# irap-omp/deconv3d

Hardware: AMD Instinct MI355X
Metric: spaxel-updates/sec (MH-Gibbs) (higher is better)
Workload: dtype f64; 1 GPU; c3_300x300x128; fsf=moffat 11x11, lsf_taps=17, spaxels=90000, lsf=analytic MUSE stand-in (mpdaf absent), parallelism=1 chain, variance=per-voxel cube (heteroscedastic)

## Files before the change

__graft_entry__.py:

```python
import os
import subprocess
import sys

ROOT = os.path.dirname(os.path.abspath(__file__))
if ROOT not in sys.path:
    sys.path.insert(0, ROOT)
CSRC = os.path.join(ROOT, "deconv3d_amd", "csrc")


SOURCES = ["d3d_api.hip", "d3d_spatial.hip", "d3d_mh.hip", "d3d_sweep.hip", "d3d_post.hip", "d3d_region.hip", "d3d_search.hip", "d3d_prep.hip", "d3d_temper.hip", "d3d_robust.hip", "d3d_pred.hip", "d3d_noise.hip", "d3d_ctx.h", "d3d_kernels.h", "d3d_conv.h",
           "d3d_mh_small.h", "d3d_rng.h", "../../include/deconv3d_hip.h"]


def tree_source_hash():
    import hashlib
    h = hashlib.sha256()
    for name in SOURCES:
        with open(os.path.join(CSRC, name), "rb") as f:
            h.update(f.read())
    return h.hexdigest()[:16]


def _binary_hash(lib):
    code = ("import ctypes,sys; l=ctypes.CDLL(sys.argv[1]); "
            "l.d3d_source_hash.restype=ctypes.c_char_p; print(l.d3d_source_hash().decode())")
    try:
        return subprocess.check_output([sys.executable, "-c", code, lib],
                                       stderr=subprocess.DEVNULL).decode().strip()
    except (subprocess.CalledProcessError, OSError):
        return None


def build():
    env = dict(os.environ)
# ... 60 lines not shown
```

deconv3d_amd/csrc/d3d_api.hip:

```cpp
#include "d3d_ctx.h"

#include <dlfcn.h>

#define D3D_VERSION 300
#ifndef D3D_SOURCE_HASH
#define D3D_SOURCE_HASH "unknown"
#endif

namespace {
thread_local std::string g_err;
}

namespace d3dh {
int fail(int code, const char *fmt, ...) {
    char buf[512];
    va_list ap;
    va_start(ap, fmt);
    vsnprintf(buf, sizeof buf, fmt, ap);
    va_end(ap);
    g_err = buf;
    return code;
}
}

// ... 160 lines not shown
                    for (int x = xs; x - fhw < pt.dx1; x += c->fw) {
                        const bool is_real = y >= pt.y0 && y < pt.y1 && x >= pt.x0 && x < pt.x1 &&
                                             c->h_mask[(size_t)y * c->W + x];
                        if (!is_real) list.push_back(make_int4(y, x, 0, 0));
                    }
                if (pt.real[col] > 0) {
                    const long n_all_col =
                        ((long)list.size() - pt.off[col]) * (c->mh_zb ? (c->Dp + 255) / 256 : 1);
                    if (c->mh_zigzag && (ord & 1) && n_all_col > c->flow_grid) {
                        std::reverse(list.begin() + pt.off[col], list.begin() + pt.off[col] + pt.real[col]);
                        std::reverse(list.begin() + pt.off[col] + pt.real[col], list.end());
                    }
                    ++ord;
                }
                most = std::max(most, (int)list.size() - pt.off[col]);
            }
        pt.off[ncol] = (int)list.size();
        const long most_wgs = (long)most * (c->mh_zb ? (c->Dp + 255) / 256 : 1);
        pt.layers = (!c->mh_layers_forced && most_wgs < c->flow_grid / 2) ? 1 : c->mh_layers_cfg;
        const bool partitioned = c->tiled || !c->part_rects.empty();
        pt.wide = pt.layers == 1 && c->mh_wide && partitioned && c->Dp == 128 && most > 0 &&
                  most <= c->flow_grid / 4 && c->mh_defer == 1;
        pt.small = pt.layers == 1 && most_wgs < c->flow_grid / 2;
        pt.chain = false;
        pt.K = 0;
        pt.last_col = -1;
        for (int col = 0; col < ncol; ++col)
            if (pt.real[col] > 0) {
                ++pt.K;
                pt.last_col = col;
            }
#ifdef D3D_EXPERIMENTS
        if (!empty && pt.K > 0) {
            const int cus = c->flow_grid / 4;
            const int fhh_ = (c->fh - 1) / 2, fhw_ = (c->fw - 1) / 2;
            const int lx0 = ((0 - c->gx0) % c->fw + c->fw) % c->fw;
            pt.chain_sx0 = (pt.dx0 - fhw_) - ((((pt.dx0 - fhw_) - lx0) % c->fw + c->fw) % c->fw);
            pt.n_sy = (pt.dy1 - pt.dy0 + 2 * c->fh - 2) / c->fh;
            pt.n_sx = (pt.dx1 + fhw_ - 1 - pt.chain_sx0) / c->fw + 1;
            (void)fhh_;
            pt.chain_ns = c->fw * c->HL;
            const int nt = (pt.chain_ns + 63) / 64 * 64 + 64;
            const bool fh_ok = c->fh == 3 || c->fh == 5 || c->fh == 7 || c->fh == 9 || c->fh == 11;
            const double g_bytes = 4.0 * pt.K * pt.n_sy * pt.n_sx * c->Dp * 8.0;
            const size_t lds = d3d::mh_chain_lds_doubles(c->fw, c->Dp, c->N, ncol, pt.K, nt / 64 - 1) * 8;
            pt.chain = c->mh_chain_opt == 1 && c->mh_defer == 1 && c->Dp <= 256 && pt.layers == 1 &&
// ... 119 lines not shown
}

int d3dh::download_device_cube(d3d_ctx *c, const double *src, double *host) { return download_cube(c, src, host); }

namespace {

enum OptKind { OPT_LAUNCH = 0, OPT_MH = 1, OPT_TAPS = 2 };
struct OptDesc {
    const char *key, *env;
    int d3d_ctx::*field;
    OptKind kind;
    int lo, hi;
};
const OptDesc g_opts[] = {
    {"mh_defer", "D3D_MH_DEFER", &d3d_ctx::mh_defer_opt, OPT_MH, 0, 2},
    {"mh_zblocks", "D3D_MH_ZBLOCKS", &d3d_ctx::mh_zblocks, OPT_MH, 0, 1},
    {"mh_layers", "D3D_MH_LAYERS", &d3d_ctx::mh_layers_opt, OPT_MH, 0, d3d::MH_LAYERS},
    {"mh_wide", "D3D_MH_WIDE", &d3d_ctx::mh_wide, OPT_MH, 0, 1},
    {"mh_props", "D3D_MH_PROPS", &d3d_ctx::mh_props, OPT_LAUNCH, 0, 1},
    {"mh_small", "D3D_MH_SMALL", &d3d_ctx::mh_small, OPT_MH, 0, 2},
    {"halo_timing", "D3D_HALO_TIMING", &d3d_ctx::halo_timing, OPT_LAUNCH, 0, 1},
    {"mh_zigzag", "D3D_MH_ZIGZAG", &d3d_ctx::mh_zigzag, OPT_MH, 0, 1},
    {"mh_nt_ivar", "D3D_MH_NT_IVAR", &d3d_ctx::mh_nt_ivar_opt, OPT_MH, -1, 1},
    {"mh_nt", "D3D_MH_NT", &d3d_ctx::mh_nt_opt, OPT_MH, 0, 1024},
    {"uniform_ivar", "D3D_UNIFORM_IVAR", &d3d_ctx::uniform_fast_path, OPT_MH, 0, 1},
    {"conv_rows", "D3D_CONV_ROWS", &d3d_ctx::conv_rows, OPT_LAUNCH, 0, 1},
    {"conv_zb", "D3D_CONV_ZB", &d3d_ctx::conv_zb, OPT_LAUNCH, 0, 1},
    {"conv_hy", "D3D_CONV_HY", &d3d_ctx::conv_hy_opt, OPT_LAUNCH, 0, 1 << 20},
    {"spatial_sep", "D3D_SPATIAL_SEP", &d3d_ctx::spatial_sep, OPT_TAPS, 0, 1},
    {"sep_fuse", "D3D_SEP_FUSE", &d3d_ctx::sep_fuse, OPT_LAUNCH, 0, 1},
    {"spatial_mode", "D3D_SPATIAL_MODE", &d3d_ctx::march_mode, OPT_LAUNCH, 0, 3},
    {"march_hy", "D3D_MARCH_HY", &d3d_ctx::march_hy_opt, OPT_TAPS, 0, 1 << 20},
    {"zmajor", "D3D_ZMAJOR", &d3d_ctx::zmajor, OPT_LAUNCH, 0, 1},
    {"zmajor_hy", "D3D_ZMAJOR_HY", &d3d_ctx::zmajor_hy, OPT_LAUNCH, 0, 1 << 20},
    {"spectral_dense", "D3D_SPECTRAL_DENSE", &d3d_ctx::spectral_dense, OPT_LAUNCH, 0, 1},
    {"spectral_blocks", "D3D_SPECTRAL_BLOCKS", &d3d_ctx::spectral_blocks, OPT_LAUNCH, 0, 1},
    {"lines_dense", "D3D_LINES_DENSE", &d3d_ctx::lines_dense, OPT_LAUNCH, 0, 3},
    {"lines_rounds", "D3D_LINES_ROUNDS", &d3d_ctx::lines_rounds, OPT_LAUNCH, 0, 64},
    {"spatial_nt", "D3D_SPATIAL_NT", &d3d_ctx::sp_nt_opt, OPT_LAUNCH, 0, 1024},
    {"xcd_remap", "D3D_XCD_REMAP", &d3d_ctx::xcd_remap, OPT_LAUNCH, 0, 1},
    {"alt_dir", "D3D_ALT_DIR", &d3d_ctx::alt_dir, OPT_LAUNCH, 0, 1},
    {"stagger", "D3D_STAGGER", &d3d_ctx::stagger, OPT_LAUNCH, 0, 1 << 20},
    {"post_nt", "D3D_POST_NT", &d3d_ctx::post_nt, OPT_LAUNCH, 0, 1},
    {"noise_timing", "D3D_NOISE_TIMING", &d3d_ctx::noise_timing, OPT_LAUNCH, 0, 1},
#ifdef D3D_EXPERIMENTS
    {"mh_chain", "D3D_MH_CHAIN", &d3d_ctx::mh_chain_opt, OPT_MH, 0, 1},
// ... 166 lines not shown
    CTX_TRY(hipMemsetAsync(c->accepted, 0, sizeof(unsigned long long), c->stream));
    CTX_TRY(hipMemsetAsync(c->acc_map, 0, (size_t)c->HW * sizeof(unsigned), c->stream));
    CTX_TRY(hipMemsetAsync(c->mask, 1, (size_t)c->HW, c->stream));
    CTX_TRY(hipStreamSynchronize(c->stream));
#undef CTX_TRY
    c->h_mask.assign((size_t)c->HW, 1);
    c->h_user_mask.assign((size_t)c->HW, 1);
    *out = c;
    return D3D_OK;
}

int d3d_ctx_destroy(d3d_ctx *c) {
    if (!c) return D3D_OK;
    (void)hipSetDevice(c->device);
    if (c->stream) (void)hipStreamSynchronize(c->stream);
    if (c->comm && g_rccl.CommDestroy) (void)g_rccl.CommDestroy(c->comm);
    c->comm = nullptr;
    for (int b = 0; b < d3d_ctx::STREAM_NB; ++b) {
        if (c->snap_host[b]) (void)hipHostFree(c->snap_host[b]);
        if (c->snap_ready[b]) (void)hipEventDestroy(c->snap_ready[b]);
        if (c->snap_done[b]) (void)hipEventDestroy(c->snap_done[b]);
    }
    if (c->copy_stream) (void)hipStreamDestroy(c->copy_stream);
    for (hipEvent_t e : c->halo_ev) (void)hipEventDestroy(e);
    if (c->ev0) (void)hipEventDestroy(c->ev0);
    if (c->ev1) (void)hipEventDestroy(c->ev1);
    if (c->own_stream) (void)hipStreamDestroy(c->own_stream);
    delete c;
    return D3D_OK;
}

int d3d_ctx_set_stream(d3d_ctx *c, void *hip_stream) {
    NEED(c, D3D_ERR_INVALID, "ctx is NULL");
    HIP_TRY(hipStreamSynchronize(c->stream));
    c->stream = hip_stream ? (hipStream_t)hip_stream : c->own_stream;
    return D3D_OK;
}

int d3d_sync(d3d_ctx *c) {
    NEED(c, D3D_ERR_INVALID, "ctx is NULL");
    HIP_TRY(hipStreamSynchronize(c->stream));
    return D3D_OK;
}

int d3d_timer_start(d3d_ctx *c) {
    NEED(c, D3D_ERR_INVALID, "ctx is NULL");
// ... 58 lines not shown
        long n = 0;
        for (const d3d_ctx::Part &pt : c->parts) n += pt.chain ? 1 : 0;
        *value = c->have_data ? n : 0;
        return D3D_OK;
    }
    if (!strcmp(key, "search_bank_ns") || !strcmp(key, "search_kernel_ns")) {
        *value = key[7] == 'b' ? c->search_bank_ns : c->search_kernel_ns;
        return D3D_OK;
    }
    if (!strcmp(key, "prep_median_ns") || !strcmp(key, "prep_stats_ns")) {
        *value = key[5] == 'm' ? c->prep_median_ns : c->prep_stats_ns;
        return D3D_OK;
    }
    if (!strcmp(key, "noise_sums_ns") || !strcmp(key, "noise_draw_ns") || !strcmp(key, "noise_apply_ns")) {
        *value = c->noise_ns[key[6] == 's' ? 0 : key[6] == 'd' ? 1 : 2];
        return D3D_OK;
    }
    if (!strcmp(key, "device_bytes")) {
        *value = (long)d3dh::dev_bytes.load();
        return D3D_OK;
    }
    if (!strcmp(key, "mh_nt_ivar_on")) {
        *value = c->mh_nt_ivar ? 1 : 0;
        return D3D_OK;
    }
    if (!strcmp(key, "batch_layers")) {
        *value = c->batch_layers;
        return D3D_OK;
    }
    if (!strcmp(key, "lsf_fits")) {
        *value = (c->have_taps && (c->ntaps == 0 || c->lsf_dense_any)) ? 1 : 0;
        return D3D_OK;
    }
    if (!strcmp(key, "lsf_taps")) {
        *value = c->ntaps;
        return D3D_OK;
    }
    if (!strcmp(key, "spatial_path") || !strcmp(key, "spectral_path") || !strcmp(key, "stage_path")) {
        *value = key[2] == 'a' ? (key[3] == 't' ? c->spatial_path : c->stage_path) : c->spectral_path;
        return D3D_OK;
    }
    if (!strcmp(key, "small_parts")) {
        long n = 0;
        for (const d3d_ctx::Part &pt : c->parts) n += d3dh::mh_part_uses_tables(c, pt) ? 1 : 0;
        *value = c->have_data ? n : 0;
        return D3D_OK;
// ... 1308 lines not shown
```

deconv3d_amd/csrc/d3d_ctx.h:

```cpp
#pragma once
#include <hip/hip_runtime.h>
#include <rccl/rccl.h>

#include <algorithm>
#include <atomic>
#include <cmath>
#include <cstdarg>
#include <cstdio>
#include <cstdlib>
#include <cstring>
#include <mutex>
#include <new>
#include <string>
#include <utility>
#include <vector>

#include "../../include/deconv3d_hip.h"
#include "d3d_kernels.h"

#ifndef D3D_WIDE_NS
#define D3D_WIDE_NS 704
#endif
constexpr int MH_WIDE_NS = D3D_WIDE_NS;
constexpr int MH_CHAIN_NT = 768;

namespace d3dh {
int fail(int code, const char *fmt, ...);
}

#define HIP_TRY(expr)                                                                   \
    do {                                                                                \
        hipError_t e_ = (expr);                                                         \
        if (e_ != hipSuccess)                                                           \
            return d3dh::fail(D3D_ERR_HIP, "%s failed: %s (%s:%d)", #expr, hipGetErrorString(e_), \
                              __FILE__, __LINE__);                                      \
    } while (0)

#define NEED(cond, code, ...) \
    do {                      \
        if (!(cond)) return d3dh::fail(code, __VA_ARGS__); \
    } while (0)

namespace d3dh {
inline std::atomic<size_t> dev_bytes{0};
}

template <typename T>
// ... 53 lines not shown
    DevBuf<double> fsf;
    DevBuf<int> lsf_shift;
    DevBuf<double> lsf_weight;
    int ntaps = 0;
    DevBuf<double> dlog;
    DevBuf<double> hwbuf;
    DevBuf<double> scal;
    DevBuf<unsigned long long> accepted;
    DevBuf<unsigned> acc_map;
    DevBuf<int4> spx;
    std::vector<int> colour_real;
    struct Part {
        int y0 = 0, y1 = 0, x0 = 0, x1 = 0;
        int dy0 = 0, dy1 = 0, dx0 = 0, dx1 = 0;
        int phase = 0;
        int layers = 1;
        bool wide = false;
        bool small = false;
        bool chain = false;
        int chain_ns = 0, chain_sx0 = 0, n_sy = 0, n_sx = 0, K = 0;
        int last_col = -1;
        std::vector<int> off;
        std::vector<int> real;
    };
    std::vector<Part> parts;
    std::vector<int4> part_rects;
    std::vector<int> part_phase;
    int n_phases = 1;
    int pend_part = -1;
    struct HaloEntry {
        int peer = 0, what = 0;
        int sy0 = 0, sy1 = 0, sx0 = 0, sx1 = 0;
        int ry0 = 0, ry1 = 0, rx0 = 0, rx1 = 0;
        size_t send_off = 0, send_n = 0, recv_off = 0, recv_n = 0;
    };
    std::vector<std::vector<HaloEntry>> plans;
    DevBuf<double> halo_send, halo_recv;
    static constexpr int STREAM_NB = 4;
    hipStream_t copy_stream = nullptr;
    DevBuf<double> snap_dev[STREAM_NB];
    double *snap_host[STREAM_NB] = {};
    hipEvent_t snap_ready[STREAM_NB] = {}, snap_done[STREAM_NB] = {};
    ncclComm_t comm = nullptr;
    int comm_rank = -1, comm_size = 0;
    int halo_timing = 0;
    static constexpr size_t HALO_RING = 64;
    std::vector<hipEvent_t> halo_ev;
    size_t halo_ev_used = 0, halo_ev_head = 0;
    double halo_ms = 0.0;
    long halo_count = 0;
    std::vector<uint8_t> h_mask;
    std::vector<uint8_t> h_user_mask;

    d3d::LineShape line = {1, {0.0, 0.0, 0.0, 0.0}, {1.0, 0.0, 0.0, 0.0}, nullptr, 0, 0.0, 0.0};
    DevBuf<double> line_tab;
    std::vector<double> h_line_tab;
    double line_tab_flux = 0.0;
    bool have_taps = false, have_data = false, have_params = false, have_cfg = false;
    bool err_valid = false;
    double min_b[3] = {}, max_b[3] = {}, amp[3] = {};
    double ra = 0;
    uint64_t seed = 0;
    int refresh_every = 1000;
    uint32_t sweep_origin = 0;

    int mh_nt = 0, mh_maxit = 0;
    int mh_nt_opt = 0, mh_maxit_opt = -1;
    int mh_defer = 1;
    int mh_defer_opt = 1;
    int mh_zblocks = 1;
    bool mh_zb = false;
    DevBuf<double> z_part;
    DevBuf<double> z_E;
#ifdef D3D_EXPERIMENTS
    DevBuf<unsigned long long> stampbuf;
    size_t stamp_launches = 0, stamp_next = 0, stamp_stride = 0;
#endif
    bool ivar_is_uniform = false;
    double ivar_uniform = 0.0;
    int uniform_fast_path = 1;
    DevBuf<double> gbuf[4];
    int lay_n = 0, lay_cy[3] = {-1, -1, -1}, lay_cx[3] = {-1, -1, -1}, lay_g[3] = {0, 0, 0};
    int mh_layers = 2;
    int batch_layers = 0;
    bool mh_nt_ivar = false;
    int mh_nt_ivar_opt = -1;
    int mh_zigzag = 1;
    int mh_layers_opt = 0;
    int mh_layers_cfg = 2;
    bool mh_layers_forced = false;
    int mh_flow = 0;
    int flow_K = 0, flow_LY = 0, flow_LX = 0, flow_items = 0, flow_grid = 0;
    int flow_last_cy = -1, flow_last_cx = -1;
    int mh_chain_opt = 0;
    DevBuf<int2> chain_cols;
    DevBuf<unsigned> chain_flags;
    DevBuf<double> chain_G;
    unsigned chain_base = 0;
    bool chain_used = false;
    int mh_props = 1;
    DevBuf<d3d::MHProposal> props;
    long props_sweep = -1;
    int mh_prio = 0;
    int mh_small = 1;
// ... 182 lines not shown
bool post_due(const d3d_ctx *c, int s);
int post_reset(d3d_ctx *c);
int region_members(d3d_ctx *c);
bool plan_has_entries(const d3d_ctx *c, int plan);
int halo_exchange(d3d_ctx *c, int plan);
int download_device_cube(d3d_ctx *c, const double *src, double *host);

bool robust_due(const d3d_ctx *c, int s);
int robust_after_sweep(d3d_ctx *c, int s);

constexpr int NOISE_STREAMS = 1024;
bool noise_due(const d3d_ctx *c, int s);
int noise_after_sweep(d3d_ctx *c, int s);

int pred_sample(d3d_ctx *c);

void colour_residue(const d3d_ctx *c, int col, int *cy, int *cx);

void pend_clear(d3d_ctx *c);
int pend_free_buf(const d3d_ctx *c);
void pend_push(d3d_ctx *c, int cy, int cx, int g);
void fill_mh_args(d3d_ctx *c, d3d::MHArgs &P);
int launch_mh(d3d_ctx *c, const d3d::MHArgs &P, unsigned grid, uint32_t sweep);
int launch_mh_zb(d3d_ctx *c, d3d::MHArgs &P, unsigned n_items, uint32_t sweep, int layers);
int launch_mh_batch(d3d_ctx *c, const d3d::MHArgs &P, unsigned grid, uint32_t sweep, int layers);
void fill_chain_args(const d3d_ctx *c, d3d::MHChainArgs &B, bool tables);
int launch_mh_defer(d3d_ctx *c, const d3d::MHArgs &P, unsigned grid, uint32_t sweep, int layers,
                    bool wide);
int flush_pending(d3d_ctx *c);
int ensure_proposals(d3d_ctx *c, uint32_t sweep);
int ensure_tables(d3d_ctx *c, bool lines);
int ensure_ptab(d3d_ctx *c);
int launch_line_table(d3d_ctx *c, const d3d::MHArgs &P, uint32_t sweep, const d3d::MHChainArgs *chains, int R);
bool mh_small_usable(const d3d_ctx *c);
int mh_ptab_row(const d3d_ctx *c, int ly, int lx, int layer = 0);
bool mh_part_uses_tables(const d3d_ctx *c, const d3d_ctx::Part &pt);
#ifdef D3D_EXPERIMENTS
int launch_mh_chain(d3d_ctx *c, int pi, uint32_t sweep0, int n_sweeps);
#endif
int launch_apply_updates(d3d_ctx *c, const d3d::MHArgs &P, const double *rec, int n);
int launch_rtnorm(d3d_ctx *c, long n, double lo, double hi, double mu, double sigma, uint64_t seed,
                  int wave_mode, double *buf);
int launch_philox(d3d_ctx *c, long n, const uint32_t *counters, const uint32_t *keys, uint32_t *words,
                  double *pairs);
#ifdef D3D_EXPERIMENTS
int launch_mh_flow(d3d_ctx *c, uint32_t sweep);
int launch_mh_pair(d3d_ctx *c, int ka, uint32_t sweep);
#endif

int temper_round(d3d_temper *t, int64_t round);
bool ctx_is_tempered(const d3d_ctx *c);
// ... 3 lines not shown
```

deconv3d_amd/csrc/d3d_mh.hip:

```cpp
#include "d3d_ctx.h"
#include "d3d_mh_small.h"

namespace d3dh {

using namespace d3d;

void pend_clear(d3d_ctx *c) {
    c->lay_n = 0;
    c->pend_part = -1;
}

int pend_free_buf(const d3d_ctx *c) {
    for (int b = 0; b < 4; ++b) {
        bool used = false;
        for (int j = 0; j < c->lay_n; ++j) used = used || c->lay_g[j] == b;
        if (!used) return b;
    }
    return 0;
}

void pend_push(d3d_ctx *c, int cy, int cx, int g) {
    c->lay_cy[c->lay_n] = cy;
    c->lay_cx[c->lay_n] = cx;
    c->lay_g[c->lay_n] = g;
// ... 353 lines not shown
    return launch_mh_small_t<UV, 256, 2, K, 1, true, false>(c, P, grid, sweep);
}
#endif

template <bool UV>
int launch_mh_small(d3d_ctx *c, const d3d::MHArgs &P, unsigned grid, uint32_t sweep, bool wide, int layers,
                    bool full) {
    NEED(P.n_lay <= layers && layers <= 2 && P.ltab && P.props, D3D_ERR_STATE,
         "internal: k_mh_small with %d pending layers of %d", P.n_lay, layers);
#ifdef D3D_EXPERIMENTS
    if (full) return launch_mh_small_full<UV, 4>(c, P, grid, sweep, layers);
#else
    (void)full;
#endif
    NEED(layers == 1, D3D_ERR_STATE, "internal: the small form keeps one pending layer");
    if (wide) return launch_mh_small_t<UV, MH_WIDE_NS, (MH_WIDE_NS > 512 ? 6 : 8), 1>(c, P, grid, sweep);
    if (c->Dp <= 64) return launch_mh_small_t<UV, 256, 8, 1>(c, P, grid, sweep);
    if (c->Dp <= 128) return launch_mh_small_t<UV, 256, 8, 2>(c, P, grid, sweep);
    return launch_mh_small_t<UV, 256, 8, 4>(c, P, grid, sweep);
}

template <bool UV>
int launch_mh_ws(d3d_ctx *c, const d3d::MHArgs &P, unsigned grid, uint32_t sweep, int layers,
                 bool wide) {
    const bool small = UV || grid < (unsigned)c->flow_grid / 2;
    if (P.ltab && layers <= 2)
        return launch_mh_small<UV>(c, P, grid, sweep, wide, layers, !(grid < (unsigned)c->flow_grid / 2));
    if (c->Dp > 256) {
        bool ntv = false;
        if constexpr (!UV) ntv = c->mh_nt_ivar && !(grid < (unsigned)c->flow_grid / 2);
        const bool few = grid < (unsigned)c->flow_grid / 2;
        if (layers >= 2) {
            if (few) return launch_mh_ws_um<UV, 4, 2, 4, false, 512>(c, P, grid, sweep);
            if constexpr (!UV)
                if (ntv) return launch_mh_ws_um<UV, 4, 2, 4, true, 512>(c, P, grid, sweep);
            return launch_mh_ws_um<UV, 4, 2, 4, false, 512>(c, P, grid, sweep);
        }
        if (few) return launch_mh_ws_um<UV, 4, 1, 4, false, 512>(c, P, grid, sweep);
        if constexpr (!UV)
            if (ntv) return launch_mh_ws_um<UV, 1, 1, 4, true, 512>(c, P, grid, sweep);
        return launch_mh_ws_um<UV, 1, 1, 4, false, 512>(c, P, grid, sweep);
    }
    if constexpr (!UV) {
        if (c->mh_nt_ivar && !small) {
            if (layers >= 3) return launch_mh_ws_um<UV, 2, 3, 2, true>(c, P, grid, sweep);
            if (layers == 2) {
                if (c->Dp > 160) return launch_mh_ws_um<UV, 2, 2, 4, true>(c, P, grid, sweep);
                return launch_mh_ws_um<UV, 2, 2, 2, true>(c, P, grid, sweep);
            }
            return launch_mh_ws_um<UV, 1, 1, 4, true>(c, P, grid, sweep);
        }
    }
    if (layers >= 3) {
        if (small) return launch_mh_ws_um<UV, 4, 3, 2>(c, P, grid, sweep);
// ... 91 lines not shown
    for (int b = 0; b < 4; ++b) {
        bool used = b == ga;
        for (int j = 0; j < c->lay_n; ++j) used = used || c->lay_g[j] == b;
        if (!used) gb = b;
    }
    F.G_a = c->gbuf[ga];
    F.G_b = c->gbuf[gb];
    c->pair_tickets += (unsigned)(F.n_a + F.n_b);
    const bool uv = c->ivar_is_uniform && c->uniform_fast_path;
    int rc;
    if (c->Dp > 160)
        rc = uv ? launch_mh_pair_t<true, 4, 4>(c, P, F, sweep) : launch_mh_pair_t<false, 2, 4>(c, P, F, sweep);
    else
        rc = uv ? launch_mh_pair_t<true, 4, 2>(c, P, F, sweep) : launch_mh_pair_t<false, 2, 2>(c, P, F, sweep);
    if (rc) return rc;
    c->lay_n = 0;
    pend_push(c, c->flow_colour[ka + 1] / c->fw, c->flow_colour[ka + 1] % c->fw, gb);
    c->pend_part = 0;
    return 0;
}
#endif

template <bool UV>
int launch_mh_zb_t(d3d_ctx *c, const d3d::MHArgs &P, unsigned n_items, uint32_t sweep, int layers) {
    constexpr int NS = 256;
    const int db = P.z_db;
    const unsigned grid = n_items * (unsigned)P.z_nb;
    const bool few = grid < (unsigned)c->flow_grid / 2;
    auto go = [&](auto kern, int M) {
        const size_t lds =
            d3d::mh_ws_lds_doubles(NS, db / 2, db, db + 2 * d3d::LSF_RL, P.npos, M) * sizeof(double);
        hipLaunchKernelGGL(kern, dim3(grid), dim3(NS + 64), lds, c->stream, P, sweep);
    };
    const bool ntv = !UV && c->mh_nt_ivar && !few;
    const int nl = P.n_lay;
    if (layers >= 2) {
        if (few) {
            if (nl == 0) go(mh_ws_kernel<NS, UV, 4, 2, 4, 0, false, true>(d3d::line_multi(P.line), false), 2);
            else if (nl == 1) go(mh_ws_kernel<NS, UV, 4, 2, 4, 1, false, true>(d3d::line_multi(P.line), false), 2);
            else go(mh_ws_kernel<NS, UV, 4, 2, 4, 2, false, true>(d3d::line_multi(P.line), false), 2);
        } else if (ntv) {
            if constexpr (!UV) {
                if (nl == 0) go(mh_ws_kernel<NS, UV, 2, 2, 4, 0, true, true>(d3d::line_multi(P.line), false), 2);
                else if (nl == 1) go(mh_ws_kernel<NS, UV, 2, 2, 4, 1, true, true>(d3d::line_multi(P.line), false), 2);
                else go(mh_ws_kernel<NS, UV, 2, 2, 4, 2, true, true>(d3d::line_multi(P.line), false), 2);
            }
        } else {
            if (nl == 0) go(mh_ws_kernel<NS, UV, 2, 2, 4, 0, false, true>(d3d::line_multi(P.line), false), 2);
            else if (nl == 1) go(mh_ws_kernel<NS, UV, 2, 2, 4, 1, false, true>(d3d::line_multi(P.line), false), 2);
            else go(mh_ws_kernel<NS, UV, 2, 2, 4, 2, false, true>(d3d::line_multi(P.line), false), 2);
        }
    } else {
        if (nl == 0) go(mh_ws_kernel<NS, UV, 4, 1, 4, 0, false, true>(d3d::line_multi(P.line), false), 1);
        else go(mh_ws_kernel<NS, UV, 4, 1, 4, 1, false, true>(d3d::line_multi(P.line), false), 1);
    }
    HIP_TRY(hipGetLastError());
    const int nw = P.z_nb * (NS / 64);
    const size_t lds2 = ((size_t)8 * nw + 8 + 16) * sizeof(double);
    hipLaunchKernelGGL(P.prior ? &d3d::k_mh_zdecide<true> : &d3d::k_mh_zdecide<false>, dim3(n_items), dim3(256), lds2,
                       c->stream, P, sweep, NS / 64);
    HIP_TRY(hipGetLastError());
    return 0;
}

int launch_mh_zb(d3d_ctx *c, d3d::MHArgs &P, unsigned n_items, uint32_t sweep, int layers) {
    NEED(P.n_lay <= (layers >= 2 ? 2 : 1), D3D_ERR_STATE, "internal: %d pending layers for the z-blocked kernel",
         P.n_lay);
    const size_t max_items = (size_t)(c->H / c->fh + 2) * (c->W / c->fw + 2);
    NEED((size_t)n_items <= max_items, D3D_ERR_STATE, "internal: %u windows in one colour launch", n_items);
    if (!c->z_part) HIP_TRY(c->z_part.alloc(max_items * P.z_nb * 32));
    if (!c->z_E) HIP_TRY(c->z_E.alloc((size_t)2 * c->slots * c->Dp));
    P.z_part = c->z_part;
    P.z_E = c->z_E;
    if (c->ivar_is_uniform && c->uniform_fast_path) return launch_mh_zb_t<true>(c, P, n_items, sweep, layers);
    return launch_mh_zb_t<false>(c, P, n_items, sweep, layers);
}

template <bool UV>
int launch_mh_batch_t(d3d_ctx *c, const d3d::MHArgs &P, unsigned grid, uint32_t sweep, int layers) {
    constexpr int NS = 256;
    const bool few = grid < (unsigned)c->flow_grid / 2;
    if (P.ltab && layers == 1) {
        const size_t lds = d3d::mh_small_lds_doubles(NS, c->HL, c->Dp, P.npos, 1) * sizeof(double);
        auto go_small = [&](auto kern) { hipLaunchKernelGGL(kern, dim3(grid), dim3(NS), lds, c->stream, P, sweep); };
        if (P.prior) {
            if (c->Dp <= 64) go_small(d3d::k_mh_small<NS, UV, 8, 1, true, 1, false, false, true>);
            else if (c->Dp <= 128) go_small(d3d::k_mh_small<NS, UV, 8, 2, true, 1, false, false, true>);
            else go_small(d3d::k_mh_small<NS, UV, 8, 4, true, 1, false, false, true>);
        } else if (c->Dp <= 64) go_small(d3d::k_mh_small<NS, UV, 8, 1, true>);
        else if (c->Dp <= 128) go_small(d3d::k_mh_small<NS, UV, 8, 2, true>);
        else go_small(d3d::k_mh_small<NS, UV, 8, 4, true>);
        HIP_TRY(hipGetLastError());
        return 0;
    }
    auto go = [&](auto kern, int M) {
        const size_t lds = d3d::mh_ws_lds_doubles(NS, c->HL, c->Dp, c->N, P.npos, M) * sizeof(double);
        hipLaunchKernelGGL(kern, dim3(grid), dim3(NS + 64), lds, c->stream, P, sweep);
    };
// ... 2 lines not shown
        if (few) {
            if (nl == 0) go(mh_ws_kernel<NS, UV, 4, 2, 2, 0, false, false, true>(d3d::line_multi(P.line), P.prior != 0), 2);
            else if (nl == 1) go(mh_ws_kernel<NS, UV, 4, 2, 2, 1, false, false, true>(d3d::line_multi(P.line), P.prior != 0), 2);
            else go(mh_ws_kernel<NS, UV, 4, 2, 2, 2, false, false, true>(d3d::line_multi(P.line), P.prior != 0), 2);
        } else {
            if (nl == 0) go(mh_ws_kernel<NS, UV, 2, 2, 2, 0, false, false, true>(d3d::line_multi(P.line), P.prior != 0), 2);
            else if (nl == 1) go(mh_ws_kernel<NS, UV, 2, 2, 2, 1, false, false, true>(d3d::line_multi(P.line), P.prior != 0), 2);
            else go(mh_ws_kernel<NS, UV, 2, 2, 2, 2, false, false, true>(d3d::line_multi(P.line), P.prior != 0), 2);
        }
    } else {
        if (nl == 0) go(mh_ws_kernel<NS, UV, 4, 1, 4, 0, false, false, true>(d3d::line_multi(P.line), P.prior != 0), 1);
        else go(mh_ws_kernel<NS, UV, 4, 1, 4, 1, false, false, true>(d3d::line_multi(P.line), P.prior != 0), 1);
    }
    HIP_TRY(hipGetLastError());
    return 0;
}

int launch_mh_batch(d3d_ctx *c, const d3d::MHArgs &P, unsigned grid, uint32_t sweep, int layers) {
    if (c->ivar_is_uniform && c->uniform_fast_path) return launch_mh_batch_t<true>(c, P, grid, sweep, layers);
    return launch_mh_batch_t<false>(c, P, grid, sweep, layers);
}

int launch_mh_defer(d3d_ctx *c, const d3d::MHArgs &P, unsigned grid, uint32_t sweep, int layers,
                    bool wide) {
    if (c->mh_defer == 1 && c->Dp <= d3d::MH_WS_MAX_DP) {
        if (c->ivar_is_uniform && c->uniform_fast_path)
            return launch_mh_ws<true>(c, P, grid, sweep, layers, wide);
        return launch_mh_ws<false>(c, P, grid, sweep, layers, wide);
    }
    switch (c->mh_nt) {
        case 128: return launch_mh_defer_nt<128>(c, P, grid, sweep);
        case 256: return launch_mh_defer_nt<256>(c, P, grid, sweep);
        case 512: return launch_mh_defer_nt<512>(c, P, grid, sweep);
        default: return launch_mh_defer_nt<1024>(c, P, grid, sweep);
    }
}

int ensure_tables(d3d_ctx *c, bool lines) {
    if (!c->props) HIP_TRY(c->props.alloc((size_t)c->HW));
    if (lines && !c->ltab) HIP_TRY(c->ltab.alloc((size_t)c->HW * 2 * c->Dp));
    return 0;
}

int launch_line_table(d3d_ctx *c, const d3d::MHArgs &P, uint32_t sweep, const d3d::MHChainArgs *chains, int R) {
    const long n = (long)(c->oy1 - c->oy0) * (c->ox1 - c->ox0) * std::max(R, 1);
    if (n <= 0) return 0;
    const size_t lds = (size_t)4 * 2 * c->N * sizeof(double);
    hipLaunchKernelGGL(d3d::line_multi(c->line) ? &d3d::k_mh_line_table<true> : &d3d::k_mh_line_table<false>,
                       dim3((unsigned)((n + 3) / 4)), dim3(256), lds, c->stream, P, sweep, c->oy0, c->oy1,
                       c->ox0, c->ox1, c->props, c->ltab, chains, R);
    HIP_TRY(hipGetLastError());
// ... 183 lines not shown
```

deconv3d_amd/csrc/d3d_sweep.hip:

```cpp
#include "d3d_ctx.h"

using namespace d3dh;

void d3dh::colour_residue(const d3d_ctx *c, int col, int *cy, int *cx) {
    *cy = ((col / c->fw - c->gy0) % c->fh + c->fh) % c->fh;
    *cx = ((col % c->fw - c->gx0) % c->fw + c->fw) % c->fw;
}

namespace {

struct SnapQueue {
    int slot[d3d_ctx::STREAM_NB];
    int head = 0, count = 0;
};

int snap_setup(d3d_ctx *c) {
    if (c->copy_stream) return 0;
    HIP_TRY(hipStreamCreateWithFlags(&c->copy_stream, hipStreamNonBlocking));
    const size_t bytes = (size_t)c->HW * 4 * sizeof(double);
    for (int b = 0; b < d3d_ctx::STREAM_NB; ++b) {
        HIP_TRY(c->snap_dev[b].alloc((size_t)c->HW * 4));
        HIP_TRY(hipHostMalloc((void **)&c->snap_host[b], bytes, hipHostMallocDefault));
        HIP_TRY(hipEventCreateWithFlags(&c->snap_ready[b], hipEventDisableTiming));
        HIP_TRY(hipEventCreateWithFlags(&c->snap_done[b], hipEventDisableTiming));
// ... 57 lines not shown
                      d3d::MHArgs &P) {
    fill_mh_args(c, P);
    P.spx = c->spx + pt.off[col];
    P.rev = (c->mh_zigzag && (ka & 1)) ? 1 : 0;
    if (tables) P.props = c->props;
    if (tables > 1) {
        P.ltab = c->ltab;
        P.ptab = c->ptab;
        int ly, lx;
        colour_residue(c, col, &ly, &lx);
        for (int j = 0; j < 2; ++j) P.ptab_row[j] = mh_ptab_row(c, ly, lx, j);
    }
    if (layers) P.write_back = (c->lay_n >= layers) ? 1 : 0;
}

void push_colour_layer(d3d_ctx *c, int pi, int col, int g, bool wrote_back) {
    if (wrote_back) c->lay_n = 0;
    int cy, cx;
    colour_residue(c, col, &cy, &cx);
    pend_push(c, cy, cx, g);
    c->pend_part = pi;
}

struct Batch {
    d3d_ctx **cs;
    int R, layers;
    bool small;
    const d3d::MHChainArgs *dev;
};

int run_part(d3d_ctx *c, int pi, uint32_t sweep, const Batch *b = nullptr) {
    d3d_ctx::Part &pt = c->parts[pi];
    const int ncol = c->fh * c->fw;
    const int layers = b ? b->layers : pt.layers;
    d3d_ctx *const self[1] = {c};
    d3d_ctx *const *cs = b ? b->cs : self;
    const bool partitioned = c->tiled || c->parts.size() > 1;
    const bool deferred =
        c->mh_defer &&
        (!partitioned || (c->mh_defer == 1 && (c->Dp <= d3d::MH_WS_MAX_DP || c->mh_zb)));
    if (c->lay_n && (c->pend_part != pi || !deferred || c->lay_n > layers))
        if (int rc = flush_pending(c)) return rc;
#ifdef D3D_EXPERIMENTS
    if (deferred && pt.chain && !b) return launch_mh_chain(c, pi, sweep, 1);
#endif
    const bool pairs = !b && deferred && c->mh_pair && !partitioned && c->mh_defer == 1 && c->Dp <= 256 &&
                       pt.layers == 2 && c->flow_K > 1 && !c->flow_first.empty();
    const bool small = deferred && c->mh_defer == 1 && !c->mh_zb && d3dh::mh_part_uses_tables(c, pt);
    const int tables = b ? (b->small ? 2 : 0)
                         : (c->mh_props && deferred && (c->mh_zb || (pt.layers == 1 && !c->deep) || small))
                               ? (small ? 2 : 1) : 0;
    int ord = 0;
    for (int col = 0; col < ncol; ++col) {
        const int n_real = pt.real[col];
        if (n_real <= 0) continue;
        const int ka = ord++;
        if (deferred) c->pend_part = pi;
#ifdef D3D_EXPERIMENTS
        if (pairs && c->lay_n == 1 && ka + 1 < c->flow_K) {
            if (c->stampbuf) goto single;
            int rc = launch_mh_pair(c, ka, sweep);
            if (rc) return rc;
            ++col;
            while (col < ncol && pt.real[col] <= 0) ++col;
            ++ord;
            continue;
        }
    single:
#else
        (void)pairs;
#endif
        if (tables && !b)
            if (int rc = ensure_proposals(c, sweep)) return rc;
        d3d::MHArgs P;
        fill_colour_args(c, pt, col, ka, deferred ? layers : 0, tables, P);
        if (!deferred) {
            if (int rc = launch_mh(c, P, (unsigned)n_real, sweep)) return rc;
            continue;
        }
        const int n_all = pt.off[col + 1] - pt.off[col];
#ifdef D3D_EXPERIMENTS
        if (!b && c->stampbuf && c->stamp_next < c->stamp_launches && (size_t)n_all * 8 <= c->stamp_stride)
            P.stamp = c->stampbuf + (c->stamp_next++) * c->stamp_stride;
#endif
        const int g_cur = pend_free_buf(c);
        int rc;
        if (b) {
            P.batch = b->dev;
            P.b_items = n_all;
            P.b_gcur = g_cur;
            for (int j = 0; j < 3; ++j) P.b_lay_g[j] = j < c->lay_n ? c->lay_g[j] : 0;
            rc = launch_mh_batch(c, P, (unsigned)n_all * b->R, sweep, layers);
        } else {
            rc = c->mh_zb ? launch_mh_zb(c, P, (unsigned)n_all, sweep, layers)
                          : launch_mh_defer(c, P, (unsigned)n_all, sweep, layers, pt.wide);
        }
        if (rc) return rc;
        for (int r = 0; r < (b ? b->R : 1); ++r) push_colour_layer(cs[r], pi, col, g_cur, P.write_back);
    }
    return 0;
}

int run_phase(d3d_ctx *c, int phase, uint32_t sweep) {
    for (size_t pi = 0; pi < c->parts.size(); ++pi)
        if (c->parts[pi].phase == phase)
            if (int rc = run_part(c, (int)pi, sweep)) return rc;
    return 0;
}

int end_sweep(d3d_ctx *c, int s, int keep_one_in, SnapQueue &snaps, double *chain_out, double *dlog_out) {
    if (s % keep_one_in == 0 && (chain_out || dlog_out))
        if (int rc = snap_push(c, snaps, s / keep_one_in, chain_out, dlog_out)) return rc;
    if (post_due(c, s))
        if (int rc = post_sample(c)) return rc;
    if (int rc = adapt_after_sweep(c, s)) return rc;
    if (c->refresh_every > 0 && s % c->refresh_every == 0) {
        if (plan_has_entries(c, D3D_PLAN_PARAMS)) {
            NEED(c->comm, D3D_ERR_STATE, "parameter gather needs d3d_comm_init");
            if (int rc = halo_exchange(c, D3D_PLAN_PARAMS)) return rc;
        }
        if (int rc = forward_into(c, c->slot[D3D_SLOT_ERR], true)) return rc;
    }
    if (int rc = robust_after_sweep(c, s)) return rc;
    return noise_after_sweep(c, s);
}

int halo_drain_one(d3d_ctx *c) {
    const size_t at = c->halo_ev_head;
    float f = 0.f;
// ... 53 lines not shown
        if (chain_batches) {
            int last = first_sweep + n_sweeps - 1;
            for (int t = s; t <= last; ++t) {
                const bool saved = t % keep_one_in == 0 && (chain_out || dlog_out);
                const bool refresh = c->refresh_every > 0 && t % c->refresh_every == 0;
                if (saved || refresh || post_due(c, t) || robust_due(c, t) || noise_due(c, t)) {
                    last = t;
                    break;
                }
            }
            if (c->lay_n && c->pend_part != 0)
                if (int rc = flush_pending(c)) return rc;
            if (int rc = launch_mh_chain(c, 0, rs, last - s + 1)) return rc;
            s = last;
        } else if (flow) {
            c->pend_part = 0;
            int rc = launch_mh_flow(c, rs);
            if (rc) return rc;
            c->pend_part = 0;
        } else
#endif
        {
            for (int ph = 0; ph < n_phases; ++ph) {
                int rc = run_phase(c, ph, rs);
                if (rc) return rc;
                if (plan_has_entries(c, ph)) {
                    hipEvent_t ev[2] = {nullptr, nullptr};
                    if (c->halo_timing) {
                        if (c->halo_ev_used == d3d_ctx::HALO_RING)
                            if (int rc2 = halo_drain_one(c)) return rc2;
                        const size_t at = (c->halo_ev_head + c->halo_ev_used) % d3d_ctx::HALO_RING;
                        while (c->halo_ev.size() < 2 * (at + 1)) {
                            hipEvent_t e;
                            HIP_TRY(hipEventCreate(&e));
                            c->halo_ev.push_back(e);
                        }
                        ev[0] = c->halo_ev[2 * at];
                        ev[1] = c->halo_ev[2 * at + 1];
                        ++c->halo_ev_used;
                        HIP_TRY(hipEventRecord(ev[0], c->stream));
                    }
                    rc = halo_exchange(c, ph);
                    if (rc) return rc;
                    if (ev[1]) HIP_TRY(hipEventRecord(ev[1], c->stream));
                }
            }
        }
// ... 136 lines not shown
}

int d3d_mh_phase(d3d_ctx *c, int phase, int sweep) {
    NEED(c, D3D_ERR_INVALID, "ctx is NULL");
    NEED(chain_ready(c), D3D_ERR_STATE, "taps/data/parameters/mh_config not set");
    NEED(phase >= 0 && phase < D3D_PLAN_PARAMS && sweep >= 0, D3D_ERR_INVALID,
         "phase %d / sweep %d out of range", phase, sweep);
    if (int rc = begin_sweeps(c, false)) return rc;
    return run_phase(c, phase, (uint32_t)sweep + c->sweep_origin);
}

int d3d_mh_colour(d3d_ctx *c, int colour, int sweep) {
    NEED(c, D3D_ERR_INVALID, "ctx is NULL");
    NEED(chain_ready(c), D3D_ERR_STATE, "taps/data/parameters/mh_config not set");
    NEED(colour >= 0 && colour < c->fh * c->fw && sweep >= 0, D3D_ERR_INVALID,
         "colour %d / sweep %d out of range", colour, sweep);
    if (int rc = begin_sweeps(c, false)) return rc;
    if (int rc = flush_pending(c)) return rc;
    for (const d3d_ctx::Part &pt : c->parts) {
        const int n_real = pt.real[colour];
        if (n_real <= 0) continue;
        d3d::MHArgs P;
        fill_colour_args(c, pt, colour, active_ordinal(pt, colour), 0, 0, P);
        int rc = launch_mh(c, P, (unsigned)n_real, (uint32_t)sweep + c->sweep_origin);
        if (rc) return rc;
    }
    return D3D_OK;
}

}
```

Measured before the change: 18.70 million spaxel-updates/s.

## Split colour launches into row strips run concurrently on auxiliary streams

Adds a strip planner that divides lattice rows into weight-balanced horizontal strips. Within each colour row, per-strip MH kernel launches are forked onto auxiliary HIP streams with separate G buffers and joined when the colour row changes. This lets independent windows from different strips overlap, aiming at the serialized per-colour launch chain on a single stream. The cost is extra events, stream synchronisation and more launches, and correctness depends on strips not interacting within one colour row.

```diff
diff --git a/__graft_entry__.py b/__graft_entry__.py
--- a/__graft_entry__.py
+++ b/__graft_entry__.py
@@ -9,7 +9,7 @@
 
 
 SOURCES = ["d3d_api.hip", "d3d_spatial.hip", "d3d_mh.hip", "d3d_sweep.hip", "d3d_post.hip", "d3d_region.hip", "d3d_search.hip", "d3d_prep.hip", "d3d_temper.hip", "d3d_robust.hip", "d3d_pred.hip", "d3d_noise.hip", "d3d_ctx.h", "d3d_kernels.h", "d3d_conv.h",
-           "d3d_mh_small.h", "d3d_rng.h", "../../include/deconv3d_hip.h"]
+           "d3d_mh_small.h", "d3d_rng.h", "../../include/deconv3d_hip.h", "d3d_strips.h"]
 
 
 def tree_source_hash():
diff --git a/deconv3d_amd/csrc/d3d_api.hip b/deconv3d_amd/csrc/d3d_api.hip
--- a/deconv3d_amd/csrc/d3d_api.hip
+++ b/deconv3d_amd/csrc/d3d_api.hip
@@ -206,6 +206,39 @@
         pt.wide = pt.layers == 1 && c->mh_wide && partitioned && c->Dp == 128 && most > 0 &&
                   most <= c->flow_grid / 4 && c->mh_defer == 1;
         pt.small = pt.layers == 1 && most_wgs < c->flow_grid / 2;
+        pt.strips = 1;
+        pt.soff.clear();
+        pt.sreal.clear();
+        {
+            const bool uv = c->ivar_is_uniform && c->uniform_fast_path;
+            const int want = c->mh_strips_opt >= 2 ? c->mh_strips_opt
+                             : (c->mh_strips_opt == 0 && most_wgs >= c->flow_grid / 2 && !uv) ? MH_STRIPS_AUTO : 1;
+            d3d_strips::Plan plan;
+            if (want >= 2 && !empty && !partitioned && c->mh_defer == 1 && (c->Dp <= d3d::MH_WS_MAX_DP || c->mh_zb) &&
+                !d3dh::mh_part_uses_tables(c, pt) && !c->mh_chain_opt && !c->mh_flow && !c->mh_pair &&
+                d3d_strips::plan(c->H, c->fh, want, &plan)) {
+                pt.strips = plan.S;
+                pt.soff.assign((size_t)ncol * (plan.S + 1), 0);
+                pt.sreal.assign((size_t)ncol * plan.S, 0);
+                for (int col = 0; col < ncol; ++col) {
+                    const int cy = col / c->fw;
+                    auto key = [&](const int4 &e) {
+                        return 2 * d3d_strips::strip_of_row(plan, d3d_strips::lattice_row(e.x, cy, c->fh)) + (e.z ? 0 : 1);
+                    };
+                    const auto b = list.begin() + pt.off[col], e = list.begin() + pt.off[col + 1];
+                    for (auto it = b; it != e; ++it)
+                        if (key(*it) < 0) return fail(D3D_ERR_HIP, "internal: lattice row outside the strips");
+                    std::stable_sort(b, e, [&](const int4 &p, const int4 &q) { return key(p) < key(q); });
+                    int *so = &pt.soff[(size_t)col * (plan.S + 1)];
+                    for (auto it = b; it != e; ++it) {
+                        const int k = key(*it);
+                        ++so[k / 2 + 1];
+                        if (!(k & 1)) ++pt.sreal[(size_t)col * plan.S + k / 2];
+                    }
+                    for (int s = 0; s < plan.S; ++s) so[s + 1] += so[s];
+                }
+            }
+        }
         pt.chain = false;
         pt.K = 0;
         pt.last_col = -1;
@@ -371,6 +404,7 @@
     {"halo_timing", "D3D_HALO_TIMING", &d3d_ctx::halo_timing, OPT_LAUNCH, 0, 1},
     {"mh_zigzag", "D3D_MH_ZIGZAG", &d3d_ctx::mh_zigzag, OPT_MH, 0, 1},
     {"mh_nt_ivar", "D3D_MH_NT_IVAR", &d3d_ctx::mh_nt_ivar_opt, OPT_MH, -1, 1},
+    {"mh_strips", "D3D_MH_STRIPS", &d3d_ctx::mh_strips_opt, OPT_MH, 0, d3d_strips::MAX_STRIPS},
     {"mh_nt", "D3D_MH_NT", &d3d_ctx::mh_nt_opt, OPT_MH, 0, 1024},
     {"uniform_ivar", "D3D_UNIFORM_IVAR", &d3d_ctx::uniform_fast_path, OPT_MH, 0, 1},
     {"conv_rows", "D3D_CONV_ROWS", &d3d_ctx::conv_rows, OPT_LAUNCH, 0, 1},
@@ -583,6 +617,11 @@
         if (c->snap_done[b]) (void)hipEventDestroy(c->snap_done[b]);
     }
     if (c->copy_stream) (void)hipStreamDestroy(c->copy_stream);
+    for (int a = 0; a < d3d_ctx::STRIP_AUX; ++a) {
+        if (c->strip_stream[a]) (void)hipStreamDestroy(c->strip_stream[a]);
+        if (c->strip_join[a]) (void)hipEventDestroy(c->strip_join[a]);
+    }
+    if (c->strip_fork) (void)hipEventDestroy(c->strip_fork);
     for (hipEvent_t e : c->halo_ev) (void)hipEventDestroy(e);
     if (c->ev0) (void)hipEventDestroy(c->ev0);
     if (c->ev1) (void)hipEventDestroy(c->ev1);
@@ -687,6 +726,10 @@
     }
     if (!strcmp(key, "mh_nt_ivar_on")) {
         *value = c->mh_nt_ivar ? 1 : 0;
+        return D3D_OK;
+    }
+    if (!strcmp(key, "mh_strips_on")) {
+        *value = (c->have_data && c->parts.size() == 1 && c->parts[0].strips > 1) ? c->parts[0].strips : 0;
         return D3D_OK;
     }
     if (!strcmp(key, "batch_layers")) {
diff --git a/deconv3d_amd/csrc/d3d_ctx.h b/deconv3d_amd/csrc/d3d_ctx.h
--- a/deconv3d_amd/csrc/d3d_ctx.h
+++ b/deconv3d_amd/csrc/d3d_ctx.h
@@ -17,12 +17,14 @@
 
 #include "../../include/deconv3d_hip.h"
 #include "d3d_kernels.h"
+#include "d3d_strips.h"
 
 #ifndef D3D_WIDE_NS
 #define D3D_WIDE_NS 704
 #endif
 constexpr int MH_WIDE_NS = D3D_WIDE_NS;
 constexpr int MH_CHAIN_NT = 768;
+constexpr int MH_STRIPS_AUTO = 2;
 
 namespace d3dh {
 int fail(int code, const char *fmt, ...);
@@ -122,6 +124,9 @@
         int last_col = -1;
         std::vector<int> off;
         std::vector<int> real;
+        int strips = 1;
+        std::vector<int> soff;
+        std::vector<int> sreal;
     };
     std::vector<Part> parts;
     std::vector<int4> part_rects;
@@ -141,6 +146,10 @@
     DevBuf<double> snap_dev[STREAM_NB];
     double *snap_host[STREAM_NB] = {};
     hipEvent_t snap_ready[STREAM_NB] = {}, snap_done[STREAM_NB] = {};
+    static constexpr int STRIP_AUX = 3;
+    hipStream_t strip_stream[STRIP_AUX] = {};
+    hipEvent_t strip_fork = nullptr, strip_join[STRIP_AUX] = {};
+    int mh_strips_opt = 0;
     ncclComm_t comm = nullptr;
     int comm_rank = -1, comm_size = 0;
     int halo_timing = 0;
@@ -179,7 +188,8 @@
     bool ivar_is_uniform = false;
     double ivar_uniform = 0.0;
     int uniform_fast_path = 1;
-    DevBuf<double> gbuf[4];
+    static constexpr int GBUFS = 8;
+    DevBuf<double> gbuf[GBUFS];
     int lay_n = 0, lay_cy[3] = {-1, -1, -1}, lay_cx[3] = {-1, -1, -1}, lay_g[3] = {0, 0, 0};
     int mh_layers = 2;
     int batch_layers = 0;
@@ -408,11 +418,12 @@
 void pend_push(d3d_ctx *c, int cy, int cx, int g);
 void fill_mh_args(d3d_ctx *c, d3d::MHArgs &P);
 int launch_mh(d3d_ctx *c, const d3d::MHArgs &P, unsigned grid, uint32_t sweep);
-int launch_mh_zb(d3d_ctx *c, d3d::MHArgs &P, unsigned n_items, uint32_t sweep, int layers);
+int launch_mh_zb(d3d_ctx *c, d3d::MHArgs &P, unsigned n_items, uint32_t sweep, int layers, unsigned total = 0,
+                 unsigned item0 = 0);
 int launch_mh_batch(d3d_ctx *c, const d3d::MHArgs &P, unsigned grid, uint32_t sweep, int layers);
 void fill_chain_args(const d3d_ctx *c, d3d::MHChainArgs &B, bool tables);
 int launch_mh_defer(d3d_ctx *c, const d3d::MHArgs &P, unsigned grid, uint32_t sweep, int layers,
-                    bool wide);
+                    bool wide, unsigned total = 0);
 int flush_pending(d3d_ctx *c);
 int ensure_proposals(d3d_ctx *c, uint32_t sweep);
 int ensure_tables(d3d_ctx *c, bool lines);
diff --git a/deconv3d_amd/csrc/d3d_mh.hip b/deconv3d_amd/csrc/d3d_mh.hip
--- a/deconv3d_amd/csrc/d3d_mh.hip
+++ b/deconv3d_amd/csrc/d3d_mh.hip
@@ -399,14 +399,14 @@
 
 template <bool UV>
 int launch_mh_ws(d3d_ctx *c, const d3d::MHArgs &P, unsigned grid, uint32_t sweep, int layers,
-                 bool wide) {
-    const bool small = UV || grid < (unsigned)c->flow_grid / 2;
+                 bool wide, unsigned total) {
+    const bool few = total < (unsigned)c->flow_grid / 2;
+    const bool small = UV || few;
     if (P.ltab && layers <= 2)
-        return launch_mh_small<UV>(c, P, grid, sweep, wide, layers, !(grid < (unsigned)c->flow_grid / 2));
+        return launch_mh_small<UV>(c, P, grid, sweep, wide, layers, !few);
     if (c->Dp > 256) {
         bool ntv = false;
-        if constexpr (!UV) ntv = c->mh_nt_ivar && !(grid < (unsigned)c->flow_grid / 2);
-        const bool few = grid < (unsigned)c->flow_grid / 2;
+        if constexpr (!UV) ntv = c->mh_nt_ivar && !few;
         if (layers >= 2) {
             if (few) return launch_mh_ws_um<UV, 4, 2, 4, false, 512>(c, P, grid, sweep);
             if constexpr (!UV)
@@ -544,11 +544,11 @@
 #endif
 
 template <bool UV>
-int launch_mh_zb_t(d3d_ctx *c, const d3d::MHArgs &P, unsigned n_items, uint32_t sweep, int layers) {
+int launch_mh_zb_t(d3d_ctx *c, const d3d::MHArgs &P, unsigned n_items, uint32_t sweep, int layers, unsigned total) {
     constexpr int NS = 256;
     const int db = P.z_db;
     const unsigned grid = n_items * (unsigned)P.z_nb;
-    const bool few = grid < (unsigned)c->flow_grid / 2;
+    const bool few = total * (unsigned)P.z_nb < (unsigned)c->flow_grid / 2;
     auto go = [&](auto kern, int M) {
         const size_t lds =
             d3d::mh_ws_lds_doubles(NS, db / 2, db, db + 2 * d3d::LSF_RL, P.npos, M) * sizeof(double);
@@ -585,17 +585,20 @@
     return 0;
 }
 
-int launch_mh_zb(d3d_ctx *c, d3d::MHArgs &P, unsigned n_items, uint32_t sweep, int layers) {
+int launch_mh_zb(d3d_ctx *c, d3d::MHArgs &P, unsigned n_items, uint32_t sweep, int layers, unsigned total,
+                 unsigned item0) {
+    if (!total) total = n_items;
     NEED(P.n_lay <= (layers >= 2 ? 2 : 1), D3D_ERR_STATE, "internal: %d pending layers for the z-blocked kernel",
          P.n_lay);
     const size_t max_items = (size_t)(c->H / c->fh + 2) * (c->W / c->fw + 2);
-    NEED((size_t)n_items <= max_items, D3D_ERR_STATE, "internal: %u windows in one colour launch", n_items);
+    NEED((size_t)item0 + n_items <= max_items, D3D_ERR_STATE, "internal: %u windows in one colour launch",
+         item0 + n_items);
     if (!c->z_part) HIP_TRY(c->z_part.alloc(max_items * P.z_nb * 32));
     if (!c->z_E) HIP_TRY(c->z_E.alloc((size_t)2 * c->slots * c->Dp));
-    P.z_part = c->z_part;
+    P.z_part = c->z_part + (size_t)item0 * P.z_nb * 32;
     P.z_E = c->z_E;
-    if (c->ivar_is_uniform && c->uniform_fast_path) return launch_mh_zb_t<true>(c, P, n_items, sweep, layers);
-    return launch_mh_zb_t<false>(c, P, n_items, sweep, layers);
+    if (c->ivar_is_uniform && c->uniform_fast_path) return launch_mh_zb_t<true>(c, P, n_items, sweep, layers, total);
+    return launch_mh_zb_t<false>(c, P, n_items, sweep, layers, total);
 }
 
 template <bool UV>
@@ -644,11 +647,12 @@
 }
 
 int launch_mh_defer(d3d_ctx *c, const d3d::MHArgs &P, unsigned grid, uint32_t sweep, int layers,
-                    bool wide) {
+                    bool wide, unsigned total) {
+    if (!total) total = grid;
     if (c->mh_defer == 1 && c->Dp <= d3d::MH_WS_MAX_DP) {
         if (c->ivar_is_uniform && c->uniform_fast_path)
-            return launch_mh_ws<true>(c, P, grid, sweep, layers, wide);
-        return launch_mh_ws<false>(c, P, grid, sweep, layers, wide);
+            return launch_mh_ws<true>(c, P, grid, sweep, layers, wide, total);
+        return launch_mh_ws<false>(c, P, grid, sweep, layers, wide, total);
     }
     switch (c->mh_nt) {
         case 128: return launch_mh_defer_nt<128>(c, P, grid, sweep);
diff --git a/deconv3d_amd/csrc/d3d_strips.h b/deconv3d_amd/csrc/d3d_strips.h
--- /dev/null
+++ b/deconv3d_amd/csrc/d3d_strips.h
@@ -0,0 +1,64 @@
+#pragma once
+
+namespace d3d_strips {
+
+constexpr int MAX_STRIPS = 4;
+constexpr int MIN_ROWS = 2;
+constexpr int ROWS_BEGIN = -1;
+
+struct Plan {
+    int S = 0;
+    int first[MAX_STRIPS + 1] = {};
+};
+
+inline int rows_end(int H, int fh) { return (H - 1 + (fh - 1) / 2) / fh + 1; }
+
+inline int lattice_row(int y, int cy, int fh) {
+    const int d = y - cy;
+    return d >= 0 ? d / fh : -((-d + fh - 1) / fh);
+}
+
+inline long row_weight(int H, int fh, int i) {
+    const int fhh = (fh - 1) / 2;
+    long w = 0;
+    for (int cy = 0; cy < fh; ++cy) {
+        const int y = cy + fh * i;
+        const int lo = y - fhh > 0 ? y - fhh : 0, hi = y + fhh < H - 1 ? y + fhh : H - 1;
+        if (hi >= lo) w += hi - lo + 1;
+    }
+    return w;
+}
+
+inline bool plan(int H, int fh, int S, Plan *out) {
+    *out = Plan();
+    if (H < 1 || fh < 1 || S < 2 || S > MAX_STRIPS) return false;
+    const int end = rows_end(H, fh);
+    if (end - ROWS_BEGIN < MIN_ROWS * S) return false;
+    long total = 0;
+    for (int i = ROWS_BEGIN; i < end; ++i) total += row_weight(H, fh, i);
+    out->first[0] = ROWS_BEGIN;
+    long cum = 0;
+    int at = ROWS_BEGIN;
+    for (int s = 1; s < S; ++s) {
+        const int lo = out->first[s - 1] + MIN_ROWS, hi = end - MIN_ROWS * (S - s);
+        while (at < lo) cum += row_weight(H, fh, at++);
+        while (at < hi) {
+            const long w = row_weight(H, fh, at);
+            if (2 * S * (cum + w) - 2 * s * total > 2 * s * total - 2 * S * cum) break;
+            cum += w;
+            ++at;
+        }
+        out->first[s] = at;
+    }
+    out->first[S] = end;
+    out->S = S;
+    return true;
+}
+
+inline int strip_of_row(const Plan &p, int i) {
+    for (int s = 0; s < p.S; ++s)
+        if (i >= p.first[s] && i < p.first[s + 1]) return s;
+    return -1;
+}
+
+}
diff --git a/deconv3d_amd/csrc/d3d_sweep.hip b/deconv3d_amd/csrc/d3d_sweep.hip
--- a/deconv3d_amd/csrc/d3d_sweep.hip
+++ b/deconv3d_amd/csrc/d3d_sweep.hip
@@ -103,6 +103,68 @@
     c->pend_part = pi;
 }
 
+int launch_real(d3d_ctx *c, const d3d_ctx::Part &pt, int col, const d3d::MHArgs &P, uint32_t sweep) {
+    if (pt.strips <= 1) return launch_mh(c, P, (unsigned)pt.real[col], sweep);
+    for (int s = 0; s < pt.strips; ++s) {
+        const int n = pt.sreal[(size_t)col * pt.strips + s];
+        if (n <= 0) continue;
+        d3d::MHArgs Ps = P;
+        Ps.spx = P.spx + pt.soff[(size_t)col * (pt.strips + 1) + s];
+        if (int rc = launch_mh(c, Ps, (unsigned)n, sweep)) return rc;
+    }
+    return 0;
+}
+
+struct StripScope {
+    d3d_ctx *c;
+    hipStream_t main;
+    int S = 1, row = -1;
+    unsigned locked = 0;
+    int setup() {
+        if (c->strip_fork) return 0;
+        for (int b = 4; b < d3d_ctx::GBUFS; ++b) {
+            HIP_TRY(c->gbuf[b].alloc((size_t)c->slots * c->Dp));
+            HIP_TRY(hipMemsetAsync(c->gbuf[b], 0, (size_t)c->slots * c->Dp * sizeof(double), main));
+        }
+        HIP_TRY(hipEventCreateWithFlags(&c->strip_fork, hipEventDisableTiming));
+        for (int a = 0; a < d3d_ctx::STRIP_AUX; ++a) {
+            HIP_TRY(hipStreamCreateWithFlags(&c->strip_stream[a], hipStreamNonBlocking));
+            HIP_TRY(hipEventCreateWithFlags(&c->strip_join[a], hipEventDisableTiming));
+        }
+        return 0;
+    }
+    int free_buf() const {
+        for (int b = 0; b < d3d_ctx::GBUFS; ++b) {
+            bool used = (locked >> b) & 1;
+            for (int j = 0; j < c->lay_n; ++j) used = used || c->lay_g[j] == b;
+            if (!used) return b;
+        }
+        return 0;
+    }
+    int fork(int strips, int colour_row, unsigned locked_bufs) {
+        if (int rc = setup()) return rc;
+        locked = locked_bufs;
+        HIP_TRY(hipEventRecord(c->strip_fork, main));
+        for (int a = 0; a + 1 < strips; ++a) HIP_TRY(hipStreamWaitEvent(c->strip_stream[a], c->strip_fork, 0));
+        S = strips;
+        row = colour_row;
+        return 0;
+    }
+    int join() {
+        c->stream = main;
+        const int n = S;
+        S = 1;
+        row = -1;
+        locked = 0;
+        for (int a = 0; a + 1 < n; ++a) {
+            HIP_TRY(hipEventRecord(c->strip_join[a], c->strip_stream[a]));
+            HIP_TRY(hipStreamWaitEvent(main, c->strip_join[a], 0));
+        }
+        return 0;
+    }
+    ~StripScope() { (void)join(); }
+};
+
 struct Batch {
     d3d_ctx **cs;
     int R, layers;
@@ -110,7 +172,7 @@
     const d3d::MHChainArgs *dev;
 };
 
-int run_part(d3d_ctx *c, int pi, uint32_t sweep, const Batch *b = nullptr) {
+int run_part(d3d_ctx *c, int pi, uint32_t sweep, const Batch *b = nullptr, bool strips_allowed = false) {
     d3d_ctx::Part &pt = c->parts[pi];
     const int ncol = c->fh * c->fw;
     const int layers = b ? b->layers : pt.layers;
@@ -131,6 +193,12 @@
     const int tables = b ? (b->small ? 2 : 0)
                          : (c->mh_props && deferred && (c->mh_zb || (pt.layers == 1 && !c->deep) || small))
                                ? (small ? 2 : 1) : 0;
+    bool strips_ok = strips_allowed && !b && pt.strips > 1 && deferred && !partitioned && c->mh_defer == 1 && tables < 2 &&
+                     (c->mh_zb || c->Dp <= d3d::MH_WS_MAX_DP);
+#ifdef D3D_EXPERIMENTS
+    strips_ok = strips_ok && !c->stampbuf && !pairs;
+#endif
+    StripScope strips = {c, c->stream};
     int ord = 0;
     for (int col = 0; col < ncol; ++col) {
         const int n_real = pt.real[col];
@@ -156,10 +224,38 @@
         d3d::MHArgs P;
         fill_colour_args(c, pt, col, ka, deferred ? layers : 0, tables, P);
         if (!deferred) {
-            if (int rc = launch_mh(c, P, (unsigned)n_real, sweep)) return rc;
+            if (int rc = launch_real(c, pt, col, P, sweep)) return rc;
             continue;
         }
         const int n_all = pt.off[col + 1] - pt.off[col];
+        if (strips.S > 1 && col / c->fw != strips.row)
+            if (int rc = strips.join()) return rc;
+        if (strips_ok && strips.S == 1) {
+            int cy, cx;
+            colour_residue(c, col, &cy, &cx);
+            unsigned locked = 0;
+            for (int j = 0; j < c->lay_n; ++j)
+                if (c->lay_cy[j] != cy) locked |= 1u << c->lay_g[j];
+            if (int rc = strips.fork(pt.strips, col / c->fw, locked)) return rc;
+        }
+        if (strips.S > 1) {
+            const int g_cur = strips.free_buf();
+            P.Gcur = c->gbuf[g_cur];
+            const int *so = &pt.soff[(size_t)col * (pt.strips + 1)];
+            for (int s = 0; s < pt.strips; ++s) {
+                const int n = so[s + 1] - so[s];
+                if (n <= 0) continue;
+                d3d::MHArgs Ps = P;
+                Ps.spx = P.spx + so[s];
+                c->stream = s ? c->strip_stream[s - 1] : strips.main;
+                const int rc = c->mh_zb ? launch_mh_zb(c, Ps, (unsigned)n, sweep, layers, (unsigned)n_all, (unsigned)so[s])
+                                        : launch_mh_defer(c, Ps, (unsigned)n, sweep, layers, pt.wide, (unsigned)n_all);
+                c->stream = strips.main;
+                if (rc) return rc;
+            }
+            push_colour_layer(c, pi, col, g_cur, P.write_back);
+            continue;
+        }
 #ifdef D3D_EXPERIMENTS
         if (!b && c->stampbuf && c->stamp_next < c->stamp_launches && (size_t)n_all * 8 <= c->stamp_stride)
             P.stamp = c->stampbuf + (c->stamp_next++) * c->stamp_stride;
@@ -179,13 +275,13 @@
         if (rc) return rc;
         for (int r = 0; r < (b ? b->R : 1); ++r) push_colour_layer(cs[r], pi, col, g_cur, P.write_back);
     }
-    return 0;
-}
-
-int run_phase(d3d_ctx *c, int phase, uint32_t sweep) {
+    return strips.join();
+}
+
+int run_phase(d3d_ctx *c, int phase, uint32_t sweep, bool strips_allowed = false) {
     for (size_t pi = 0; pi < c->parts.size(); ++pi)
         if (c->parts[pi].phase == phase)
-            if (int rc = run_part(c, (int)pi, sweep)) return rc;
+            if (int rc = run_part(c, (int)pi, sweep, nullptr, strips_allowed)) return rc;
     return 0;
 }
 
@@ -285,7 +381,7 @@
 #endif
         {
             for (int ph = 0; ph < n_phases; ++ph) {
-                int rc = run_phase(c, ph, rs);
+                int rc = run_phase(c, ph, rs, true);
                 if (rc) return rc;
                 if (plan_has_entries(c, ph)) {
                     hipEvent_t ev[2] = {nullptr, nullptr};
@@ -468,7 +564,7 @@
         if (n_real <= 0) continue;
         d3d::MHArgs P;
         fill_colour_args(c, pt, colour, active_ordinal(pt, colour), 0, 0, P);
-        int rc = launch_mh(c, P, (unsigned)n_real, (uint32_t)sweep + c->sweep_origin);
+        int rc = launch_real(c, pt, colour, P, (uint32_t)sweep + c->sweep_origin);
         if (rc) return rc;
     }
     return D3D_OK;
```

After: 19.62 million spaxel-updates/s (median of 6 runs). 4.9% higher.
